# KatanaMajesty/Nebulae

Hardware: AMD Instinct MI355X
Metric: denoised frames/s (1920x1080: GI 1 spp + SVGF temporal + a-trous) (higher is better)
Workload: dtype f32

## Files before the change

### nebulae_amd/csrc/gi.hip

```cpp
#include "gi_device.h"

namespace neb {

#ifndef NEB_SORT_BITS
#define NEB_SORT_BITS 16
#endif
constexpr int kSortBits = NEB_SORT_BITS;
static_assert(kSortBits >= 1 && kSortBits <= 16, "raysort.hip sorts at most two 8-bit digits");

__device__ __forceinline__ uint32_t bounce_sort_key(float3 o, float3 d, const float* smin, const float* sinv)
{
    const uint32_t oct = (d.x < 0.f ? 1u : 0u) | (d.y < 0.f ? 2u : 0u) | (d.z < 0.f ? 4u : 0u);
    const uint32_t key = (oct << (kSortBits - 3)) | (morton30(o, smin, sinv) >> (30 - (kSortBits - 3)));
    return min(key, (1u << kSortBits) - 2u);
}

struct GiRecords {
    float4* ray_o;
    float4* ray_d;
    float4* hit;
    float4* path;
    float4* state;
    float4* srec;
};
constexpr int kSrO = 0, kSrD = 1, kSrContrib = 2, kSrSum = 3;

struct GiArgs {
    SceneView S;
    neb_gi_constants c;
    GiRecords R;
    const uint32_t* albedo;
    const uint32_t* rough_metal;
    const uint2* world_pos;
    const uint2* normal;
    float4* radiance;
    neb_gi_hit* hits;
    unsigned long long* ray_counter;
    uint32_t* bounce_counts;
    uint32_t* shadow_counts;
    uint32_t* table_counts;
    uint32_t sun_table;
    uint32_t hint_pairs;
    uint32_t W, row_begin, row0, row1, tiles_x;
    uint32_t sample;
    uint32_t bounce;
    uint32_t stats;
    uint32_t defer_resolve;
    const uint32_t* tile_order;
    uint32_t* sort_keys;
    uint32_t* sort_vals;
    const uint32_t* sort_order;
    uint32_t* bsort_keys;
    uint32_t* bsort_vals;
    uint32_t raygen_only;
    float4* list;
    uint32_t* list_counts;
    uint32_t list_cap, list_set;
    float smin[3], sinv[3];
    uint32_t first_px, n_px;
};
template <uint32_t RUNS>
__device__ __forceinline__ uint32_t gi_block()
{
    if constexpr (RUNS == 0u)
        return blockIdx.x;
    const uint32_t seg_len = ((gridDim.x + RUNS - 1u) / RUNS + 7u) & ~7u;
    const uint32_t seg = blockIdx.x / seg_len, b = blockIdx.x - seg * seg_len;
    const uint32_t n = min(seg_len, gridDim.x - seg * seg_len);
    const uint32_t q = n >> 3, r = n & 7u, xcd = b & 7u, k = b >> 3;
    return seg * seg_len + (xcd < r ? xcd * (q + 1u) + k : r * (q + 1u) + (xcd - r) * q + k);
}
constexpr uint32_t kShadeRuns = 16u, kRaygenRuns = 16u;
constexpr uint32_t kListSegments = 128u;
#ifndef NEB_LIST_QUAD_BELOW
#define NEB_LIST_QUAD_BELOW 1500000u
#endif
#ifndef NEB_LIST_WAVES
#define NEB_LIST_WAVES 6
#endif

template <uint32_t RUNS = 0u>
__device__ __forceinline__ bool gi_pixel(const GiArgs& a, uint32_t& x, uint32_t& y, size_t& i)
{
    const uint32_t lane = threadIdx.x;
    const uint32_t blk = gi_block<RUNS>();
    const uint32_t tile_x = blk % a.tiles_x, tile_y = blk / a.tiles_x;
    x = tile_x * 8 + (lane & 7);
    y = a.row0 + tile_y * 8 + (lane >> 3);
    i = (size_t)(y - a.row_begin) * a.W + x;
    return x < a.W && y < a.row1;
}

__device__ __forceinline__ void count_rays(uint32_t* block_counts, uint32_t mine, uint32_t slot)
{
    uint32_t total = mine;
#pragma unroll
    for (int off = 32; off > 0; off >>= 1)
        total += __shfl_down(total, off);
    if ((threadIdx.x & 63u) == 0 && total)
        block_counts[slot] += total;
}
__device__ __forceinline__ void count_rays(uint32_t* block_counts, uint32_t mine) { count_rays(block_counts, mine, blockIdx.x); }

#ifndef NEB_RG_STACK
#define NEB_RG_STACK 12
#endif
constexpr int kRgStack = NEB_RG_STACK;
static_assert(32 * (kRgStack * 256 + 1024) <= 160 * 1024 || NEB_TRACE_WAVES < 8, "LDS budget of the closest-hit pass: 32 waves per CU of stacks and child slots in 160 KB");
__global__ __launch_bounds__(64, NEB_TRACE_WAVES) void gi_raygen_trace_kernel(GiArgs a)
{
    __shared__ int stack_mem[kRgStack * 64];
    __shared__ __attribute__((aligned(16))) int child_slot_mem[256];
// ... 74 lines not shown
    count_rays(a.bounce_counts, rays);
    if (a.stats) {
#pragma unroll
        for (int k = 0; k < 5; ++k) {
            uint32_t v = wave_stamp[k];
#pragma unroll
            for (int off = 32; off > 0; off >>= 1)
                v = max(v, (uint32_t)__shfl_xor((int)v, off));
            if (lane == 0)
                atomicAdd(a.ray_counter + 6 + k, (unsigned long long)v);
        }
        if (lane == 0)
            atomicAdd(a.ray_counter + 5, 1ull);
    }
}

__global__ __launch_bounds__(64, NEB_TRACE_WAVES) void gi_bounce_trace_kernel(GiArgs a)
{
    __shared__ int stack_mem[kLdsStack * 64];
    uint32_t x, y;
    size_t i = 0;
    bool active;
    if (a.sort_order) {
        const uint32_t j = blockIdx.x * 64u + threadIdx.x;
        active = j < a.n_px;
        if (active)
            i = a.sort_order[j];
    } else {
        active = gi_pixel(a, x, y, i);
    }
    uint32_t rays = 0;
    if (active) {
        const float4 rd = a.R.ray_d[i];
        if (rd.w != 0.0f) {
            const float4 ro = a.R.ray_o[i];
            Hit hit;
            rays = 1;
            float4 h = make_float4(-1.0f, 0.f, 0.f, 0.f);
            if (traverse(a.S, f3(ro.x, ro.y, ro.z), f3(rd.x, rd.y, rd.z), ro.w, kTraceMax, false, stack_mem + threadIdx.x, hit))
                h = make_float4(hit.t, hit.u, hit.v, __uint_as_float(hit.tri));
            a.R.hit[i] = h;
        }
    }
    if (a.bounce > 1)
        count_rays(a.bounce_counts, rays);
}

struct ShadeOut {
    float4 rec_o = {0.f, 0.f, 0.f, 0.f}, shadow_d = {0.f, 0.f, 0.f, 0.f} , rec_c = {0.f, 0.f, 0.f, 0.f}, sum = {0.f, 0.f, 0.f, 0.f};
    uint32_t rays = 0;
    uint32_t table = 0;
};

template <bool FAST, bool STAGED>
__device__ __forceinline__ void shade_pixel(const GiArgs& a, size_t i, const float4 h, ShadeOut& o, const float4* staged, uint32_t staged_swz)
{
    const float4 pth = a.R.path[i];
    const float4 rd = a.R.ray_d[i];
    const uint32_t trav_iters = a.stats ? __float_as_uint(a.R.srec[4 * i + kSrContrib].w) : 0u;
    float3 throughput = f3(pth.x, pth.y, pth.z);
    if (!(a.sample == 0 && a.bounce == 1))
        o.sum = a.R.srec[4 * i + kSrSum];
    float4 next_d = make_float4(0.f, 0.f, 0.f, 0.f);
    neb_gi_hit dbg = {-1.0f, ~0u, ~0u, 0u};
    const bool alive = rd.w != 0.0f;
    if (alive && h.x == -1.0f) {
        o.sum.x += a.c.skyColor[0] * throughput.x;
        o.sum.y += a.c.skyColor[1] * throughput.y;
        o.sum.z += a.c.skyColor[2] * throughput.z;
    } else if (alive && h.x >= 0.0f) {
        const uint32_t tri = __float_as_uint(h.w);
        Surface surf;
        uint32_t geom;
        TriShade ts;
        if constexpr (STAGED)
            ts = load_tri_shade_at(staged, staged_swz);
        else
            ts = load_tri_shade(a.S, tri);
        const bool shaded = reconstruct_surface<FAST>(a.S, ts, h.y, h.z, surf, geom);
        dbg.t = h.x;
        dbg.geometry = geom;
        if (a.hits)
            dbg.primitive = __float_as_uint(a.S.shade[8 * (size_t)tri + 7].x);
        if (shaded) {
            const float4 ro = a.R.ray_o[i];
            const float3 org = f3(ro.x, ro.y, ro.z), dir = f3(rd.x, rd.y, rd.z);
            const float3 hitP = org + dir * h.x;
            const float3 V = normalize3<FAST>(-dir);
            uint32_t rng = __float_as_uint(pth.w);
            const float a0 = rand01(rng), a1 = rand01(rng);
            const float angle = a0 * 2.0f * 3.1415926535f, dist = fsqrt<false>(a1);
            const float3 sun_dir = f3(a.c.sunLightDirection[0], a.c.sunLightDirection[1], a.c.sunLightDirection[2]);
            const float3 sun_rad = f3(a.c.sunLightRadiance[0], a.c.sunLightRadiance[1], a.c.sunLightRadiance[2]);
            const float3 L = normalize3<false>(-sun_dir);
            const float3 Bv = normalize3<false>(perpendicular(L));
            const float3 T = cross3(Bv, L);
            float sn_a, cs_a;
            det_sincosf(angle, sn_a, cs_a);
            const float3 inc = normalize3<false>(L + (Bv * sn_a + T * cs_a) * a.c.sunTanHalfAngle * dist);
            const bool transition = dot3(surf.GN, inc) <= 0.0f;
            const float3 so = hitP + (transition ? -surf.GN : surf.GN) * 1e-2f;
            const float3 O = evaluate_direct_brdf<FAST>(surf, V, L) * sun_rad * throughput;
            o.rays = 1;
            const uint32_t side = transition ? 1u : 0u;
            bool hinted_hit = false;
            if (a.sun_table && !((ts.lit >> side) & 1u) && ts.hint_side == side && ts.hint[0] != kNoHint) {
                float tt, uu, vv;
#pragma unroll
                for (int pair = 0; pair < kHints && !hinted_hit; pair += 2) {
                    const uint32_t h0 = ts.hint[pair];
                    if (h0 == kNoHint || (uint32_t)pair >= 2u * a.hint_pairs)
                        break;
                    const uint32_t h1 = ts.hint[pair + 1] != kNoHint ? ts.hint[pair + 1] : h0;
                    const float4 a0 = a.S.tris[3 * h0], b0 = a.S.tris[3 * h0 + 1], c0 = a.S.tris[3 * h0 + 2];
                    const float4 a1 = a.S.tris[3 * h1], b1 = a.S.tris[3 * h1 + 1], c1 = a.S.tris[3 * h1 + 2];
                    hinted_hit = intersect_tri_regs(a0, b0, c0, so, inc, 0.001f, kTraceMax, tt, uu, vv) ||
                                 intersect_tri_regs(a1, b1, c1, so, inc, 0.001f, kTraceMax, tt, uu, vv);
                }
            }
            if (hinted_hit) {
                o.table = 1;
            } else if (a.sun_table && ((ts.lit >> side) & 1u)) {
                o.sum.x += O.x;
                o.sum.y += O.y;
                o.sum.z += O.z;
                o.table = 1;
                dbg.flags |= 1u;
            } else {
                o.rec_o = make_float4(so.x, so.y, so.z, 0.001f);
                o.shadow_d = make_float4(inc.x, inc.y, inc.z, 1.0f);
                o.rec_c = make_float4(O.x, O.y, O.z, 0.f);
            }
            if (a.bounce + 1 < a.c.maxPathVertices) {
                uint32_t rng_copy = rng;
                const float3 SNn = normalize3<FAST>(surf.SN);
                const float e0 = rand01(rng_copy), e1 = rand01(rng_copy);
                const float3 Ld = cosine_hemisphere_aligned<FAST>(e0, e1, SNn);
                const float pdiff = 1.0f - specular_probability<FAST>(saturate1(dot3(V, SNn)), specular_f0(surf.albedo, surf.metalness), surf.albedo);
                const float3 no = hitP + surf.GN * 1e-2f;
                throughput = throughput * (surf.albedo * (1.0f - surf.metalness));
                if (rand01(rng) < pdiff)
                    throughput = f3(fdiv<FAST>(throughput.x, pdiff), fdiv<FAST>(throughput.y, pdiff), fdiv<FAST>(throughput.z, pdiff));
                a.R.ray_o[i] = make_float4(no.x, no.y, no.z, 0.001f);
                next_d = make_float4(Ld.x, Ld.y, Ld.z, 1.0f);
                a.R.path[i] = make_float4(throughput.x, throughput.y, throughput.z, __uint_as_float(rng));
            }
            if (a.sample + 1 < a.c.samplesPerPixel)
                a.R.state[i] = make_float4(V.x, V.y, V.z, __uint_as_float(rng));
        }
    }
    if (a.bounce + 1 < a.c.maxPathVertices)
        a.R.ray_d[i] = next_d;
    if (a.sort_keys) {
        uint32_t key = (1u << kSortBits) - 1u;
        if (o.shadow_d.w != 0.0f) {
            key = min(morton30(f3(o.rec_o.x, o.rec_o.y, o.rec_o.z), a.smin, a.sinv) >> (30 - kSortBits), (1u << kSortBits) - 2u);
        }
        a.sort_keys[i] = key;
        a.sort_vals[i] = (uint32_t)i;
    }
    if (a.bsort_keys) {
        uint32_t key = (1u << kSortBits) - 1u;
        if (next_d.w != 0.0f) {
            const float4 no4 = a.R.ray_o[i];
            key = bounce_sort_key(f3(no4.x, no4.y, no4.z), f3(next_d.x, next_d.y, next_d.z), a.smin, a.sinv);
        }
        a.bsort_keys[i] = key;
        a.bsort_vals[i] = (uint32_t)i;
    }
    if (a.hits && a.bounce == 1) {
        if (a.stats)
            dbg.flags |= min(trav_iters, 4095u) << 8;
        a.hits[i] = dbg;
    }
}

template <bool FAST>
__global__ __launch_bounds__(64, NEB_SHADE_WAVES) void gi_shade_kernel(GiArgs a)
{
    uint32_t x, y;
    size_t i;
    const bool active = gi_pixel<kShadeRuns>(a, x, y, i);
    ShadeOut o;
    float4 h = make_float4(-2.0f, 0.f, 0.f, 0.f);
    if (active)
        h = a.R.hit[i];
    __shared__ float4 smem[64 * 8];
    const uint32_t lane = threadIdx.x;
    const bool has_hit = active && h.x >= 0.0f;
    const uint32_t my_tri = has_hit ? __float_as_uint(h.w) : ~0u;
#pragma unroll
    for (uint32_t it = 0; it < 8; ++it) {
        const uint32_t src = it * 8u + (lane >> 3);
        const uint32_t t = (uint32_t)__shfl((int)my_tri, (int)src);
        if (t != ~0u) {
            const float4* g = a.S.shade + 8 * (size_t)t + ((lane & 7u) ^ (src & 7u));
            __builtin_amdgcn_global_load_lds((const __attribute__((address_space(1))) void*)g, (__attribute__((address_space(3))) void*)(smem + it * 64u), 16, 0, 0);
        }
    }
    __syncthreads();
    if (active)
        shade_pixel<FAST, true>(a, i, h, o, smem + lane * 8u, lane & 7u);
    if (a.list) {
        const bool trace = active && o.shadow_d.w != 0.0f;
        const bool final_vertex = a.sample + 1 == a.c.samplesPerPixel && a.bounce + 1 >= a.c.maxPathVertices && !a.defer_resolve;
        if (active && !trace) {
            if (final_vertex) {
                if (o.sum.x != 0.0f || o.sum.y != 0.0f || o.sum.z != 0.0f) {
                    const float inv_spp = 1.0f / (float)a.c.samplesPerPixel;
                    float4 r = a.radiance[i];
                    r.x += o.sum.x * inv_spp;
                    r.y += o.sum.y * inv_spp;
                    r.z += o.sum.z * inv_spp;
                    a.radiance[i] = r;
                }
            } else {
                a.R.srec[4 * i + kSrSum] = o.sum;
            }
        }
        const unsigned long long m = __ballot(trace);
        if (m) {
            const uint32_t seg = blockIdx.x % kListSegments;
            uint32_t base = 0;
            if (lane == 0)
                base = atomicAdd(a.list_counts + a.list_set * kListSegments + seg, (uint32_t)__popcll(m));
            base = (uint32_t)__shfl((int)base, 0);
            if (trace) {
                const uint32_t slot = base + (uint32_t)__popcll(m & ((1ull << lane) - 1ull));
                float4* rec = a.list + 4 * ((size_t)seg * a.list_cap + slot);
                rec[kSrO] = make_float4(o.rec_o.x, o.rec_o.y, o.rec_o.z, __uint_as_float((uint32_t)i));
                rec[kSrD] = o.shadow_d;
                rec[kSrContrib] = o.rec_c;
                rec[kSrSum] = o.sum;
            }
        }
        count_rays(a.shadow_counts, o.rays);
        count_rays(a.table_counts, o.table);
        return;
    }
    __syncthreads();
    float4* xpose = smem;
    xpose[lane * 4 + kSrO] = o.rec_o;
    xpose[lane * 4 + kSrD] = o.shadow_d;
    xpose[lane * 4 + kSrContrib] = o.rec_c;
    xpose[lane * 4 + kSrSum] = o.sum;
    __syncthreads();
    const uint32_t blk = gi_block<kShadeRuns>();
    const uint32_t tile_x = blk % a.tiles_x, tile_y = blk / a.tiles_x;
#pragma unroll
    for (uint32_t k = 0; k < 4; ++k) {
        const uint32_t row = 2 * k + (lane >> 5), col = (lane & 31u) >> 2, comp = lane & 3u;
        const uint32_t px = tile_x * 8 + col, py = a.row0 + tile_y * 8 + row;
        if (px < a.W && py < a.row1)
            a.R.srec[4 * ((size_t)(py - a.row_begin) * a.W + px) + comp] = xpose[(row * 8 + col) * 4 + comp];
    }
    count_rays(a.shadow_counts, o.rays);
    count_rays(a.table_counts, o.table);
}

__device__ __forceinline__ void shadow_wave(const GiArgs& a, size_t i, bool valid, int* stack_mem)
{
    float4* stage = reinterpret_cast<float4*>(stack_mem);
    const uint32_t lane = threadIdx.x;
// ... 356 lines not shown
    GiState::DispatchSet& ds = g->sets[phase == 1 ? (g->begun & 1u) : phase == 2 ? (g->finished & 1u) : g->defer_resolve == 2 ? (g->traces & 1u) : 0u];
    if (g->debug_hits && !g->d_hits) {
        void* p = nullptr;
        GI_HIP(ctx, hipMalloc(&p, npx * sizeof(neb_gi_hit)));
        GI_HIP(ctx, hipMemset(p, 0, npx * sizeof(neb_gi_hit)));
        g->allocs.push_back(p);
        g->d_hits = (neb_gi_hit*)p;
    }
    if (!ds.d_records) {
        void* p = nullptr;
        GI_HIP(ctx, hipMalloc(&p, npx * sizeof(float4) * 9));
        g->allocs.push_back(p);
        ds.d_records = (float4*)p;
    }
    GiArgs a;
    a.S = g->view;
    a.c = *c;
    a.R.ray_o = ds.d_records;
    a.R.ray_d = ds.d_records + npx;
    a.R.hit = ds.d_records + 2 * npx;
    a.R.path = ds.d_records + 3 * npx;
    a.R.state = ds.d_records + 4 * npx;
    a.R.srec = ds.d_records + 5 * npx;
    a.albedo = (const uint32_t*)ctx->planes[NEB_PLANE_ALBEDO][0];
    a.rough_metal = (const uint32_t*)ctx->planes[NEB_PLANE_ROUGH_METAL][0];
    a.world_pos = (const uint2*)ctx->planes[NEB_PLANE_WORLDPOS][0];
    a.normal = (const uint2*)ctx->planes[NEB_PLANE_NORMAL][ctx->cur];
    a.radiance = (float4*)ctx->planes[NEB_PLANE_RADIANCE][ctx->cur];
    a.hits = g->debug_hits ? g->d_hits : nullptr;
    a.ray_counter = g->d_ray_counter;
    a.W = ctx->W;
    a.row_begin = ctx->row_begin;
    a.row0 = row0;
    a.row1 = row1;
    a.tiles_x = (ctx->W + 7) / 8;
    a.stats = g->debug_hits ? 1u : 0u;
    a.sort_keys = a.sort_vals = nullptr;
    a.sort_order = nullptr;
    a.tile_order = (g->d_tile_order && g->tile_order_n == a.tiles_x * ((row1 - row0 + 7) / 8)) ? g->d_tile_order : nullptr;
    a.first_px = (uint32_t)((size_t)(row0 - ctx->row_begin) * ctx->W);
    a.n_px = (uint32_t)((size_t)(row1 - row0) * ctx->W);
    for (int q = 0; q < 3; ++q) {
        a.smin[q] = g->scene_min[q];
        a.sinv[q] = 1.0f / fmaxf(g->scene_max[q] - g->scene_min[q], 1e-20f);
    }
    a.bsort_keys = a.bsort_vals = nullptr;
    a.raygen_only = 0;
    if (phase != 1) {
        GI_HIP(ctx, gi_sun_table_update(g, *c, (hipStream_t)stream));
        GI_HIP(ctx, gi_sun_table_order(g, (hipStream_t)stream));
        g->last_dispatch_stream = (hipStream_t)stream;
        g->last_dispatch_stream_set = true;
    }
    a.sun_table = g->sun_table_state == 1 ? 1u : 0u;
    a.hint_pairs = (uint32_t)g->sun_hints / 2u;
    int tail_slot = -1;
    bool tail_warm = false;
    if (a.sun_table && g->compact_shadow && g->tail_tune && phase != 1) {
        if (g->tail_phase == 3 && hipEventQuery(g->tail_ev[1]) == hipSuccess && hipEventQuery(g->tail_ev[3]) == hipSuccess) {
            float ms_lists = 0.f, ms_sorted = 0.f;
            if (hipEventElapsedTime(&ms_lists, g->tail_ev[0], g->tail_ev[1]) == hipSuccess && hipEventElapsedTime(&ms_sorted, g->tail_ev[2], g->tail_ev[3]) == hipSuccess) {
                g->tail_us[0] = ms_lists * 1e3f, g->tail_us[1] = ms_sorted * 1e3f;
                g->tail_sorted = ms_sorted < 0.95f * ms_lists;
            }
            g->tail_phase = 0;
        } else if (g->tail_phase == 1 && !ds.d_list) {
        } else if (g->tail_phase == 2 && !ds.d_sort && (g->sort_shadow_auto ? a.n_px >= 1500000u : g->sort_shadow)) {
            tail_warm = true;
        } else if (g->tail_phase == 1 || g->tail_phase == 2) {
            tail_slot = g->tail_phase == 1 ? 0 : 2;
            for (int k = 0; k < 2; ++k)
                if (!g->tail_ev[tail_slot + k])
                    GI_HIP(ctx, hipEventCreate(&g->tail_ev[tail_slot + k]));
            g->tail_phase++;
        }
        (void)hipGetLastError();
    }
    const bool compact = a.sun_table && g->compact_shadow && !tail_warm && (tail_slot >= 0 ? tail_slot == 0 : !g->tail_sorted);
    const bool sort_shadow = !compact && (g->sort_shadow_auto ? a.n_px >= 1500000u : g->sort_shadow);
    if (sort_shadow || g->sort_bounce) {
        if (!ds.d_sort) {
            void* p = nullptr;
            GI_HIP(ctx, hipMalloc(&p, 8 * npx * sizeof(uint32_t)));
            g->allocs.push_back(p);
            ds.d_sort = (uint32_t*)p;
            const size_t bytes = ray_sort_scratch_bytes(npx);
            GI_HIP(ctx, hipMalloc(&p, bytes));
            g->allocs.push_back(p);
            ds.d_sort_temp = p;
            g->sort_temp_bytes = bytes;
        }
        if (sort_shadow) {
            a.sort_keys = ds.d_sort;
            a.sort_vals = ds.d_sort + npx;
        }
        if (g->sort_bounce) {
            a.bsort_keys = ds.d_sort + 4 * npx;
            a.bsort_vals = ds.d_sort + 5 * npx;
            a.raygen_only = 1;
        }
    }
    a.defer_resolve = g->defer_resolve ? 1u : 0u;
    ds.pending_spp = c->samplesPerPixel;
    ds.pending_row0 = row0;
    ds.pending_row1 = row1;
    if (g->defer_resolve == 2)
// ... 487 lines not shown
```

### nebulae_amd/csrc/gi_build.hip

```cpp
#include <cstring>
#include <rocprim/device/device_radix_sort.hpp>
#include <rocprim/device/device_scan.hpp>

#include <algorithm>
#include <chrono>
#include <cstdlib>

#include "gi_device.h"

namespace neb {

void gi_on_resize(GiState* g)
{
    if (!g)
        return;
    std::vector<void*> stale = {g->d_hits, g->d_direct_counts};
    for (GiState::DispatchSet& ds : g->sets) {
        for (void* p : {(void*)ds.d_records, (void*)ds.d_block_counts, (void*)ds.d_sort, ds.d_sort_temp, (void*)ds.d_list})
            stale.push_back(p);
        ds = GiState::DispatchSet{};
    }
    g->traces = g->resolves = 0;
    g->begun = g->finished = 0;
    for (void* p : stale) {
// ... 1166 lines not shown
        if (standalone[i]) {
            if (table_entries + (size_t)dtexs[i].w * dtexs[i].h > 0xfffffffeull) {
                delete g;
                return gi_fail(ctx, NEB_ERR_OUT_OF_RANGE, "neb_gi_set_scene: more than 2^32 texels in standalone texture tables");
            }
            dtexs[i].offset = (uint32_t)table_entries;
            table_entries += (size_t)dtexs[i].w * dtexs[i].h;
        }
    g->texture_table_bytes = table_entries * 16 + bundle_entries * 32;
    {
        uint32_t* d_raw = nullptr;
        uint4* d_tables = nullptr;
        uint4* d_bundles = nullptr;
        hipError_t te = hipSuccess;
        auto talloc = [&](void** p, size_t bytes, bool keep) {
            if (te != hipSuccess)
                return;
            te = hipMalloc(p, bytes ? bytes : 16);
            if (te == hipSuccess && keep)
                g->allocs.push_back(*p);
        };
        talloc((void**)&d_raw, raw_total * 4, false);
        talloc((void**)&d_tables, table_entries * 16, true);
        talloc((void**)&d_bundles, bundle_entries * 32, true);
        for (uint32_t i = 0; i < n_texs && te == hipSuccess; ++i)
            te = hipMemcpy(d_raw + raw_off[i], texs[i].rgba8, (size_t)texs[i].width * texs[i].height * 4, hipMemcpyHostToDevice);
        for (uint32_t i = 0; i < n_texs && te == hipSuccess; ++i)
            if (standalone[i]) {
                const size_t n_pos = (size_t)dtexs[i].w * dtexs[i].h;
                hipLaunchKernelGGL(texture_footprints_kernel, dim3((unsigned)((n_pos + 255) / 256)), dim3(256), 0, nullptr, d_raw + raw_off[i],
                                   dtexs[i].w, dtexs[i].h, d_tables + dtexs[i].offset, 1u);
                te = hipGetLastError();
            }
        for (uint32_t i = 0; i < n_mats && te == hipSuccess; ++i) {
            const DevMat& d = dmats[i];
            if (!d.bundle_w)
                continue;
            const size_t n_pos = (size_t)d.bundle_w * d.bundle_h;
            hipLaunchKernelGGL(material_bundle_kernel, dim3((unsigned)((n_pos + 255) / 256)), dim3(256), 0, nullptr, d_raw + raw_off[d.tex[0]],
                               d_raw + raw_off[d.tex[1]], d_raw + raw_off[d.tex[2]], d.bundle_w, d.bundle_h, d_bundles + 2 * (size_t)d.bundle);
            te = hipGetLastError();
        }
        if (te == hipSuccess)
            te = hipDeviceSynchronize();
        if (d_raw)
            (void)hipFree(d_raw);
        if (te != hipSuccess) {
            gi_destroy(g);
            return gi_fail(ctx, NEB_ERR_HIP, "neb_gi_set_scene: texture tables", te);
        }
        g->view.texels = reinterpret_cast<const uint32_t*>(d_tables);
        g->view.bundles = d_bundles;
    }
    g->n_tris = (uint32_t)(g->h_tris.size() / 12);
    memcpy(g->scene_min, smin, sizeof(smin));
    memcpy(g->scene_max, smax, sizeof(smax));
    hipError_t e = hipSuccess;
    if ((e = upload(g, dgeoms, &g->view.geoms)) != hipSuccess || (e = upload(g, dmats, &g->view.mats)) != hipSuccess ||
        (e = upload(g, dtexs, &g->view.texs)) != hipSuccess || (e = upload(g, indices, &g->view.indices)) != hipSuccess ||
        (e = upload(g, normals, &g->view.normals)) != hipSuccess || (e = upload(g, uvs, &g->view.uvs)) != hipSuccess ||
        (e = upload(g, tangents, &g->view.tangents)) != hipSuccess) {
        gi_destroy(g);
        return gi_fail(ctx, NEB_ERR_HIP, "neb_gi_set_scene: upload", e);
    }
    void* ctr = nullptr;
    if ((e = hipMalloc(&ctr, 16 * sizeof(unsigned long long))) != hipSuccess || (e = hipMemset(ctr, 0, 16 * sizeof(unsigned long long))) != hipSuccess) {
        gi_destroy(g);
        return gi_fail(ctx, NEB_ERR_HIP, "neb_gi_set_scene: counter", e);
    }
    g->allocs.push_back(ctr);
    g->d_ray_counter = (unsigned long long*)ctr;
    g->view.n_tris = g->n_tris;
    ctx->gi = g;
    return NEB_OK;
}

#ifndef NEB_SPLIT_AREA_FACTOR
#define NEB_SPLIT_AREA_FACTOR 16.0
#endif
constexpr double kSplitAreaFactor = NEB_SPLIT_AREA_FACTOR, kSplitBudget = 0.25;

struct HostRef {
    uint32_t tri;
    float lo[3], hi[3];
    bool clipped;
};

static double half_area(const float lo[3], const float hi[3])
{
    const double dx = (double)hi[0] - lo[0], dy = (double)hi[1] - lo[1], dz = (double)hi[2] - lo[2];
    return dx * dy + dy * dz + dz * dx;
}

static bool clipped_bounds(const float* t, const float lo[3], const float hi[3], float out_lo[3], float out_hi[3])
{
    double poly[16][3], tmp[16][3];
    int n = 3;
    for (int c = 0; c < 3; ++c) {
        poly[0][c] = t[c];
        poly[1][c] = (double)t[c] + t[3 + c];
        poly[2][c] = (double)t[c] + t[6 + c];
    }
    for (int axis = 0; axis < 3 && n > 0; ++axis)
        for (int side = 0; side < 2 && n > 0; ++side) {
            const double plane = side == 0 ? (double)lo[axis] : (double)hi[axis], sgn = side == 0 ? 1.0 : -1.0;
            int m = 0;
            for (int i = 0; i < n; ++i) {
                const int j = (i + 1) % n;
                const double di = sgn * (poly[i][axis] - plane), dj = sgn * (poly[j][axis] - plane);
                if (di >= 0.0) {
                    for (int c = 0; c < 3; ++c)
                        tmp[m][c] = poly[i][c];
                    ++m;
                }
// ... 469 lines not shown
```

### nebulae_amd/csrc/gi_device.h

```cpp
#pragma once
#pragma clang fp contract(off)

#include "gi_internal.h"

namespace neb {

__device__ __forceinline__ float3 f3(float x, float y, float z) { return make_float3(x, y, z); }
__device__ __forceinline__ float3 operator+(float3 a, float3 b) { return f3(a.x + b.x, a.y + b.y, a.z + b.z); }
__device__ __forceinline__ float3 operator-(float3 a, float3 b) { return f3(a.x - b.x, a.y - b.y, a.z - b.z); }
__device__ __forceinline__ float3 operator*(float3 a, float s) { return f3(a.x * s, a.y * s, a.z * s); }
__device__ __forceinline__ float3 operator*(float3 a, float3 b) { return f3(a.x * b.x, a.y * b.y, a.z * b.z); }
__device__ __forceinline__ float3 operator-(float3 a) { return f3(-a.x, -a.y, -a.z); }
__device__ __forceinline__ float dot3(float3 a, float3 b) { return a.x * b.x + a.y * b.y + a.z * b.z; }
__device__ __forceinline__ float3 cross3(float3 a, float3 b)
{
    return f3(a.y * b.z - a.z * b.y, a.z * b.x - a.x * b.z, a.x * b.y - a.y * b.x);
}
template <bool FAST> __device__ __forceinline__ float fdiv(float a, float b) { return FAST ? a * __builtin_amdgcn_rcpf(b) : a / b; }
template <bool FAST> __device__ __forceinline__ float fsqrt(float x) { return FAST ? __builtin_amdgcn_sqrtf(x) : sqrtf(x); }
__device__ __forceinline__ void det_sincosf(float x, float& s, float& c)
{
    const float k = rintf(x * 0.636619772367581343f);
    float r = fmaf(-k, 1.57079637050628662109375f, x);
    r = fmaf(-k, -4.37113900018624283e-8f, r);
// ... 83 lines not shown
    int e;
    const float m = frexpf(f, &e);
    e -= 1;
    if (e > 15)
        return max_bits;
    if (e < -14)
        return (uint32_t)rintf(ldexpf(f, 14 + mbits));
    const float q = rintf(ldexpf(2.0f * m - 1.0f, mbits));
    const uint32_t bits = ((uint32_t)(e + 15) << mbits) + (uint32_t)q;
    return bits > max_bits ? max_bits : bits;
}
__device__ __forceinline__ float3 unpack_r11g11b10(uint32_t v)
{
    return f3(small_float_decode(v & 0x7ffu, 6), small_float_decode((v >> 11) & 0x7ffu, 6),
              small_float_decode((v >> 22) & 0x3ffu, 5));
}

__device__ __forceinline__ float luminance3(float3 c) { return c.x * 0.2126f + c.y * 0.7152f + c.z * 0.0722f; }
__device__ __forceinline__ float3 specular_f0(float3 albedo, float metal)
{
    return f3(lerp1(0.04f, albedo.x, metal), lerp1(0.04f, albedo.y, metal), lerp1(0.04f, albedo.z, metal));
}
template <bool FAST = false> __device__ __forceinline__ float3 fresnel_schlick(float3 f0, float vdoth)
{
    const float k = 1.0f - fpow5<FAST>(vdoth);
    return f3(f0.x + (1.0f - f0.x) * k, f0.y + (1.0f - f0.y) * k, f0.z + (1.0f - f0.z) * k);
}
template <bool FAST = false> __device__ __forceinline__ float specular_probability(float vdotn, float3 f0, float3 albedo)
{
    const float dr = luminance3(albedo);
    const float fres = saturate1(luminance3(fresnel_schlick<FAST>(f0, saturate1(vdotn))));
    const float diff = dr * (1.0f - fres);
    const float p = fdiv<FAST>(diff, fmaxf(0.0001f, fres + diff));
    return fminf(fmaxf(p, 0.1f), 0.9f);
}
template <bool FAST = false> __device__ __forceinline__ float3 cosine_hemisphere_aligned(float u0, float u1, float3 sn)
{
    const float a = fsqrt<FAST>(u0), b = kPiTwo * u1;
    float sb, cb;
    det_sincosf(b, sb, cb);
    const float3 z = f3(a * cb, a * sb, fsqrt<FAST>(1.0f - u0));
    const float3 up = fabsf(sn.z) < 0.999f ? f3(0, 0, 1) : f3(1, 0, 0);
    const float3 tx = normalize3<FAST>(cross3(up, sn));
    const float3 ty = cross3(sn, tx);
    return normalize3<FAST>(tx * z.x + ty * z.y + sn * z.z);
}
__device__ __forceinline__ float3 perpendicular(float3 u)
{
    const float3 a = f3(fabsf(u.x), fabsf(u.y), fabsf(u.z));
    const uint32_t xm = ((a.x - a.y) < 0 && (a.x - a.z) < 0) ? 1 : 0;
    const uint32_t ym = (a.y - a.z) < 0 ? (1 ^ xm) : 0;
    const uint32_t zm = 1 ^ (xm | ym);
    return cross3(u, f3((float)xm, (float)ym, (float)zm));
}

struct Surface {
    float3 GN, SN, albedo;
    float roughness, metalness;
};

template <bool FAST = false> __device__ float3 evaluate_direct_brdf(const Surface& s, float3 V, float3 L)
{
    const float3 N = s.SN;
    const float3 Hv = normalize3<FAST>(V + L);
    const float LdotN = dot3(L, N), VdotH = saturate1(dot3(V, Hv)), VdotN = dot3(V, N), NdotH = dot3(N, Hv);
    const float3 F0 = specular_f0(s.albedo, s.metalness);
    const float3 F = fresnel_schlick<FAST>(F0, saturate1(VdotH));
    const float3 Kd = f3(1.0f - F.x, 1.0f - F.y, 1.0f - F.z);
    const float3 diff = Kd * (s.albedo * kPiInv);
    const float vn = saturate1(VdotN), ln = saturate1(LdotN), nh = saturate1(NdotH);
    float3 spec = f3(0, 0, 0);
    const float den = 4.0f * vn * ln;
    if (den > 0.0f) {
        const float alpha = s.roughness * s.roughness;
        const float a2 = alpha * alpha;
        const float dd = (nh * nh) * (a2 - 1.0f) + 1.0f;
        const float ndf = fdiv<FAST>(a2, kPi * dd * dd);
        const float k = alpha * 0.5f;
        const float gv = vn * fdiv<FAST>(1.0f, vn * (1.0f - k) + k);
        const float gl = ln * fdiv<FAST>(1.0f, ln * (1.0f - k) + k);
        const float c = ndf * (gv * gl);
        const float inv = fdiv<FAST>(1.0f, den);
        spec = f3(c * F.x * inv, c * F.y * inv, c * F.z * inv);
    }
    return diff + spec;
}

#ifndef NEB_LDS_STACK
#define NEB_LDS_STACK 16
#endif
constexpr int kLdsStack = NEB_LDS_STACK;
constexpr int kSpillStack = 64 - kLdsStack;
static_assert((kLdsStack + kSpillStack) / 3 == 21, "GiState::max_bvh_depth assumes a 64-entry traversal stack");

struct Hit {
    float t, u, v;
    uint32_t tri;
    uint32_t node_visits, tri_tests;
    uint32_t w_iters, w_node_iters, w_node_lanes, w_leaf_iters, w_leaf_lanes;
    uint32_t top_visits[4], deep_sp;
};

__device__ __forceinline__ bool intersect_tri_regs(float4 a, float4 b, float4 c, float3 o, float3 d, float tmin, float tmax, float& t,
                                                   float& u, float& v)
{
    const float3 v0 = f3(a.x, a.y, a.z), e1 = f3(a.w, b.x, b.y), e2 = f3(b.z, b.w, c.x);
// ... 425 lines not shown
            };
            const float a = un(top.x, top.y), b = un(top.z, top.w), cc = un(bot.x, bot.y), dd = un(bot.z, bot.w);
            const float tp = a + fx * (b - a), bt = cc + fx * (dd - cc);
            ch[c] = tp + fy * (bt - tp);
        }
        out.albedo = make_float4(ch[0], ch[1], ch[2], 0.0f);
        out.normal = make_float4(ch[3], ch[4], ch[5], 0.0f);
        out.rm = make_float4(0.0f, ch[6], ch[7], 0.0f);
        return;
    }
    if (m.tex[0] >= 0)
        out.albedo = sample_texture<FAST>(S, m.tex[0], u, v);
    if (m.tex[1] >= 0)
        out.normal = sample_texture<FAST>(S, m.tex[1], u, v);
    if (m.tex[2] >= 0)
        out.rm = sample_texture<FAST>(S, m.tex[2], u, v);
}

__device__ __forceinline__ float3 load3(const float* p, uint32_t i) { return f3(p[3 * i], p[3 * i + 1], p[3 * i + 2]); }
__device__ __forceinline__ float3 xform_dir(const float* m, float3 p)
{
    return f3(p.x * m[0] + p.y * m[3] + p.z * m[6], p.x * m[1] + p.y * m[4] + p.z * m[7], p.x * m[2] + p.y * m[5] + p.z * m[8]);
}

struct TriShade {
    float3 n0, n1, n2;
    float2 uv0, uv1, uv2;
    float4 t0, t1, t2;
    uint32_t geom;
    uint32_t lit;
    uint32_t hint[kHints], hint_side;
};
template <typename Ptr> __device__ __forceinline__ TriShade load_tri_shade_at(Ptr r, uint32_t swz)
{
    const float4 r0 = r[0 ^ swz], r1 = r[1 ^ swz], r2 = r[2 ^ swz], r6 = r[6 ^ swz];
    TriShade t;
    t.n0 = f3(r0.x, r0.y, r0.z);
    t.n1 = f3(r1.x, r1.y, r1.z);
    t.n2 = f3(r2.x, r2.y, r2.z);
    t.uv0 = make_float2(r0.w, r1.w);
    t.uv1 = make_float2(r2.w, r6.x);
    t.uv2 = make_float2(r6.y, r6.z);
    t.geom = __float_as_uint(r6.w) & kGeomMask;
    t.lit = __float_as_uint(r6.w) >> kLitShift;
    t.t0 = r[3 ^ swz];
    t.t1 = r[4 ^ swz];
    t.t2 = r[5 ^ swz];
    const float4 r7 = r[7 ^ swz];
    unpack_hints(r7, t.hint, t.hint_side);
    return t;
}
__device__ __forceinline__ TriShade load_tri_shade(const SceneView& S, uint32_t tri) { return load_tri_shade_at(S.shade + 8 * (size_t)tri, 0u); }

template <bool FAST = false> __device__ __forceinline__ bool reconstruct_surface(const SceneView& S, const TriShade& ts, float bu, float bv, Surface& out, uint32_t& geom)
{
    geom = ts.geom;
    const DevGeom g = S.geoms[geom];
    const float b0 = 1.0f - (bu + bv), b1 = bu, b2 = bv;
    if (!g.valid)
        return false;
    const float3 n0 = ts.n0, n1 = ts.n1, n2 = ts.n2;
    const float3 gn = normalize3<FAST>(f3(n0.x * b0 + n1.x * b1 + n2.x * b2, n0.y * b0 + n1.y * b1 + n2.y * b2, n0.z * b0 + n1.z * b1 + n2.z * b2));
    out.GN = normalize3<FAST>(xform_dir(g.m, gn));
    const float u = ts.uv0.x * b0 + ts.uv1.x * b1 + ts.uv2.x * b2;
    const float v = ts.uv0.y * b0 + ts.uv1.y * b1 + ts.uv2.y * b2;
    if (g.material < 0)
        return false;
    const DevMat m = S.mats[g.material];
    MapSamples maps;
    sample_material_maps<FAST>(S, m, u, v, maps);
    if (m.tex[0] < 0) {
        out.albedo = f3(m.albedo[0], m.albedo[1], m.albedo[2]);
    } else {
        const float4 t = maps.albedo;
        out.albedo = f3(t.x, t.y, t.z);
    }
    if (m.tex[1] < 0) {
        out.SN = out.GN;
    } else {
        float tg[4];
        tg[0] = ts.t0.x * b0 + ts.t1.x * b1 + ts.t2.x * b2;
        tg[1] = ts.t0.y * b0 + ts.t1.y * b1 + ts.t2.y * b2;
        tg[2] = ts.t0.z * b0 + ts.t1.z * b1 + ts.t2.z * b2;
        tg[3] = ts.t0.w * b0 + ts.t1.w * b1 + ts.t2.w * b2;
        const float l4 = fsqrt<FAST>(tg[0] * tg[0] + tg[1] * tg[1] + tg[2] * tg[2] + tg[3] * tg[3]);
#pragma unroll
        for (int k = 0; k < 4; ++k)
            tg[k] = fdiv<FAST>(tg[k], l4);
        const float3 T = f3(tg[0], tg[1], tg[2]);
        const float3 B = normalize3<FAST>(cross3(out.GN, T) * tg[3]);
        const float4 t = maps.normal;
        const float3 N = f3(t.x * 2.0f - 1.0f, t.y * 2.0f - 1.0f, t.z * 2.0f - 1.0f);
        out.SN = normalize3<FAST>(T * N.x + B * N.y + out.GN * N.z);
    }
    if (m.tex[2] < 0) {
        out.roughness = m.rough;
        out.metalness = m.metal;
    } else {
        const float4 t = maps.rm;
        out.roughness = t.y;
        out.metalness = t.z;
    }
    return true;
}

__device__ __forceinline__ uint32_t expand_bits10(uint32_t v)
{
    v = (v * 0x00010001u) & 0xFF0000FFu;
    v = (v * 0x00000101u) & 0x0F00F00Fu;
    v = (v * 0x00000011u) & 0xC30C30C3u;
    v = (v * 0x00000005u) & 0x49249249u;
    return v;
}

__device__ __forceinline__ uint32_t morton30(float3 p, const float* smin, const float* sinv)
{
    const uint32_t qx = (uint32_t)fminf(fmaxf((p.x - smin[0]) * sinv[0] * 1024.0f, 0.0f), 1023.0f);
    const uint32_t qy = (uint32_t)fminf(fmaxf((p.y - smin[1]) * sinv[1] * 1024.0f, 0.0f), 1023.0f);
    const uint32_t qz = (uint32_t)fminf(fmaxf((p.z - smin[2]) * sinv[2] * 1024.0f, 0.0f), 1023.0f);
    return (expand_bits10(qx) << 2) | (expand_bits10(qy) << 1) | expand_bits10(qz);
}
// ... 3 lines not shown
```

### nebulae_amd/csrc/gi_internal.h

```cpp
#pragma once
#include <cmath>
#include <cstdio>
#include <cstring>
#include <vector>

#include "neb_device.h"
#include "neb_internal.h"

namespace neb {


struct DevGeom {
    float m[9];
    int32_t material;
    uint32_t firstIndex;
    uint32_t vertexBase;
    uint32_t valid;
    uint32_t pad[3];
};
struct DevMat {
    int32_t tex[3];
    float albedo[3];
    float rough, metal;
    uint32_t bundle;
    uint32_t bundle_w, bundle_h;
    uint32_t pad;
};
struct DevTex {
    uint32_t offset;
    uint32_t w, h, pad;
};
struct BvhNode {
    float c0min[3];
    int32_t c0;
    float c0max[3];
    int32_t c1;
    float c1min[3];
    uint32_t pad0;
    float c1max[3];
    uint32_t pad1;
};

struct Bvh4Node {
    float4 lox, loy, loz;
    int4 child;
    float4 hix, hiy, hiz;
    int4 pad;
};
static_assert(sizeof(Bvh4Node) == 128 && offsetof(Bvh4Node, hix) == offsetof(Bvh4Node, lox) + 64, "node layout");
struct Bvh4NodeQ {
    float ox, oy, oz, sx;
    float sy, sz;
    uint32_t qlox, qloy;
    uint32_t qloz, qhix, qhiy, qhiz;
    int4 child;
};
static_assert(sizeof(Bvh4NodeQ) == 64, "quantised node layout");
#ifndef NEB_TRACE_WAVES
#define NEB_TRACE_WAVES 8
#endif
#ifndef NEB_SHADE_WAVES
#define NEB_SHADE_WAVES 4
#endif
#ifndef NEB_LEAF_BATCH
#define NEB_LEAF_BATCH 12
#endif
constexpr int kLeafBatch = NEB_LEAF_BATCH;
#ifndef NEB_MAX_LEAF_TRIS
#define NEB_MAX_LEAF_TRIS 2
#endif
constexpr int kMaxLeafTris = NEB_MAX_LEAF_TRIS;
constexpr uint32_t kLitShift = 30u, kGeomMask = (1u << kLitShift) - 1u;
constexpr int kHints = 4;
constexpr uint32_t kNoHint = 0x7fffffu;
__host__ __device__ inline void pack_hints(const uint32_t hint[kHints], uint32_t side, float4& r7)
{
    uint32_t h[kHints];
    for (int k = 0; k < kHints; ++k)
        h[k] = hint[k] < kNoHint ? hint[k] : kNoHint;
    const unsigned long long lo = (unsigned long long)h[0] | ((unsigned long long)h[1] << 23) | ((unsigned long long)(h[2] & 0x3ffffu) << 46);
    union { uint32_t u; float f; } y, z, w;
    y.u = (uint32_t)lo;
    z.u = (uint32_t)(lo >> 32);
    w.u = (h[2] >> 18) | (h[3] << 5) | (side << 31);
    r7.y = y.f, r7.z = z.f, r7.w = w.f;
}
__host__ __device__ inline void unpack_hints(const float4& r7, uint32_t hint[kHints], uint32_t& side)
{
    union { float f; uint32_t u; } y, z, w;
    y.f = r7.y, z.f = r7.z, w.f = r7.w;
    const unsigned long long lo = (unsigned long long)y.u | ((unsigned long long)z.u << 32);
    hint[0] = (uint32_t)lo & kNoHint;
    hint[1] = (uint32_t)(lo >> 23) & kNoHint;
    hint[2] = ((uint32_t)(lo >> 46) | (w.u << 18)) & kNoHint;
    hint[3] = (w.u >> 5) & kNoHint;
    side = w.u >> 31;
}

struct SceneView {
    const float4* tris;
    const Bvh4Node* nodes;
    const Bvh4NodeQ* qnodes;
    const DevGeom* geoms;
    const DevMat* mats;
    const DevTex* texs;
    const uint32_t* indices;
    const float* normals;
    const float* uvs;
    const float* tangents;
    const uint32_t* texels;
    const uint4* bundles;
    const float4* shade;
    uint32_t n_tris;
    int32_t root;
    uint32_t n_qnodes;
};

struct GiState {
    SceneView view{};
    std::vector<void*> allocs;
    std::vector<float> h_tris;
    float scene_min[3] = {0, 0, 0}, scene_max[3] = {0, 0, 0};
    uint32_t n_tris = 0, n_nodes = 0, bvh_depth = 0, build_passes = 0;
    float build_ms = 0.f;
    size_t texture_table_bytes = 0;
    uint32_t max_bvh_depth = 21;
    bool built = false;
    unsigned long long* d_ray_counter = nullptr;
    neb_gi_hit* d_hits = nullptr;
    bool debug_hits = false;
    struct DispatchSet {
        float4* d_records = nullptr;
        uint32_t* d_sort = nullptr;
        void* d_sort_temp = nullptr;
        uint32_t* d_block_counts = nullptr;
        uint32_t* d_list = nullptr;
        uint32_t list_epoch = 0;
        uint32_t pending_spp = 1, pending_row0 = 0, pending_row1 = 0;
        bool awaiting_resolve = false;
        uint32_t resolve_seq = 0;
        neb_gi_constants split_c{};
        uint32_t split_row0 = 0, split_row1 = 0;
    } sets[2];
    uint32_t resolve_seq = 0;
    uint32_t* d_tile_order = nullptr;
    uint32_t tile_order_n = 0, tile_order_cap = 0;
    uint32_t traces = 0, resolves = 0;
    uint32_t begun = 0, finished = 0;
    uint32_t* d_direct_counts = nullptr;
    unsigned long long last_stats[16] = {};
    int defer_resolve = 0;
    bool exact_shade = false;
    bool sort_shadow = true;
    bool sort_shadow_auto = true;
    bool sort_bounce = false;
    size_t sort_temp_bytes = 0;
    size_t n_block_counts = 0;
    bool sun_table = true;
    int sun_table_state = 0;
    float sun_table_pending[4] = {0, 0, 0, 0};
    uint32_t sun_hold = 2, sun_seen = 0, sun_table_age = 0;
    int sun_hold_option = 0;
    float sun_table_key[4] = {0, 0, 0, 0};
    unsigned long long* d_sun_counts = nullptr;
    uint32_t* d_sun_hint_list = nullptr;
    uint32_t sun_hint_list_cap = 0;
    uint32_t sun_table_builds = 0;
    hipEvent_t sun_table_event = nullptr;
    hipEvent_t sun_build_ev[2] = {nullptr, nullptr};
    hipStream_t sun_table_stream = nullptr;
    bool sun_table_event_pending = false;
    hipStream_t last_dispatch_stream = nullptr;
// ... 56 lines not shown
```

Measured before the change: 1640.

## Flatten geometry+material into one header and hoist shade-kernel loads

Builds a per-geometry 128-byte ShadeHeader that merges the geometry transform and its material, so shading reads it with six vector loads instead of two dependent loads (geom, then material). Path, ray direction, origin, radiance and the first hint-triangle pair are loaded earlier in the shade kernel so their latency overlaps with other work. The sun basis (L, B, T) is now computed once on the host and passed in the kernel arguments instead of per pixel. The cost is extra register pressure from the hoisted loads and a larger argument struct.

New measurement: 1702, median of 6. 1.04x the previous value.

```diff
diff --git a/nebulae_amd/csrc/gi.hip b/nebulae_amd/csrc/gi.hip
--- a/nebulae_amd/csrc/gi.hip
+++ b/nebulae_amd/csrc/gi.hip
@@ -58,6 +58,8 @@
     uint32_t list_cap, list_set;
     float smin[3], sinv[3];
     uint32_t first_px, n_px;
+    const ShadeHeader* heads;
+    float sun_L[3], sun_B[3], sun_T[3];
 };
 template <uint32_t RUNS>
 __device__ __forceinline__ uint32_t gi_block()
@@ -238,11 +240,10 @@
     uint32_t table = 0;
 };
 
-template <bool FAST, bool STAGED>
-__device__ __forceinline__ void shade_pixel(const GiArgs& a, size_t i, const float4 h, ShadeOut& o, const float4* staged, uint32_t staged_swz)
-{
-    const float4 pth = a.R.path[i];
-    const float4 rd = a.R.ray_d[i];
+template <bool FAST>
+__device__ __forceinline__ void shade_pixel(const GiArgs& a, size_t i, const float4 h, const float4 pth, const float4 rd, const float4 ro, ShadeOut& o,
+                                            const float4* staged, uint32_t staged_swz)
+{
     const uint32_t trav_iters = a.stats ? __float_as_uint(a.R.srec[4 * i + kSrContrib].w) : 0u;
     float3 throughput = f3(pth.x, pth.y, pth.z);
     if (!(a.sample == 0 && a.bounce == 1))
@@ -257,30 +258,29 @@
     } else if (alive && h.x >= 0.0f) {
         const uint32_t tri = __float_as_uint(h.w);
         Surface surf;
-        uint32_t geom;
-        TriShade ts;
-        if constexpr (STAGED)
-            ts = load_tri_shade_at(staged, staged_swz);
-        else
-            ts = load_tri_shade(a.S, tri);
-        const bool shaded = reconstruct_surface<FAST>(a.S, ts, h.y, h.z, surf, geom);
+        const TriShade ts = load_tri_shade_at(staged, staged_swz);
+        const ShadeHead head = load_shade_header(a.heads, ts.geom);
+        const bool hint_fetch = a.sun_table && a.hint_pairs && !((ts.lit >> ts.hint_side) & 1u) && ts.hint[0] != kNoHint;
+        float4 ha0 = make_float4(0.f, 0.f, 0.f, 0.f), hb0 = ha0, hc0 = ha0, ha1 = ha0, hb1 = ha0, hc1 = ha0;
+        if (hint_fetch) {
+            const uint32_t h0 = ts.hint[0], h1 = ts.hint[1] != kNoHint ? ts.hint[1] : h0;
+            ha0 = a.S.tris[3 * h0], hb0 = a.S.tris[3 * h0 + 1], hc0 = a.S.tris[3 * h0 + 2];
+            ha1 = a.S.tris[3 * h1], hb1 = a.S.tris[3 * h1 + 1], hc1 = a.S.tris[3 * h1 + 2];
+        }
+        const bool shaded = reconstruct_surface<FAST>(a.S, head, ts, h.y, h.z, surf);
         dbg.t = h.x;
-        dbg.geometry = geom;
+        dbg.geometry = ts.geom;
         if (a.hits)
             dbg.primitive = __float_as_uint(a.S.shade[8 * (size_t)tri + 7].x);
         if (shaded) {
-            const float4 ro = a.R.ray_o[i];
             const float3 org = f3(ro.x, ro.y, ro.z), dir = f3(rd.x, rd.y, rd.z);
             const float3 hitP = org + dir * h.x;
             const float3 V = normalize3<FAST>(-dir);
             uint32_t rng = __float_as_uint(pth.w);
             const float a0 = rand01(rng), a1 = rand01(rng);
             const float angle = a0 * 2.0f * 3.1415926535f, dist = fsqrt<false>(a1);
-            const float3 sun_dir = f3(a.c.sunLightDirection[0], a.c.sunLightDirection[1], a.c.sunLightDirection[2]);
             const float3 sun_rad = f3(a.c.sunLightRadiance[0], a.c.sunLightRadiance[1], a.c.sunLightRadiance[2]);
-            const float3 L = normalize3<false>(-sun_dir);
-            const float3 Bv = normalize3<false>(perpendicular(L));
-            const float3 T = cross3(Bv, L);
+            const float3 L = f3(a.sun_L[0], a.sun_L[1], a.sun_L[2]), Bv = f3(a.sun_B[0], a.sun_B[1], a.sun_B[2]), T = f3(a.sun_T[0], a.sun_T[1], a.sun_T[2]);
             float sn_a, cs_a;
             det_sincosf(angle, sn_a, cs_a);
             const float3 inc = normalize3<false>(L + (Bv * sn_a + T * cs_a) * a.c.sunTanHalfAngle * dist);
@@ -297,6 +297,11 @@
                     const uint32_t h0 = ts.hint[pair];
                     if (h0 == kNoHint || (uint32_t)pair >= 2u * a.hint_pairs)
                         break;
+                    if (pair == 0) {
+                        hinted_hit = intersect_tri_regs(ha0, hb0, hc0, so, inc, 0.001f, kTraceMax, tt, uu, vv) ||
+                                     intersect_tri_regs(ha1, hb1, hc1, so, inc, 0.001f, kTraceMax, tt, uu, vv);
+                        continue;
+                    }
                     const uint32_t h1 = ts.hint[pair + 1] != kNoHint ? ts.hint[pair + 1] : h0;
                     const float4 a0 = a.S.tris[3 * h0], b0 = a.S.tris[3 * h0 + 1], c0 = a.S.tris[3 * h0 + 2];
                     const float4 a1 = a.S.tris[3 * h1], b1 = a.S.tris[3 * h1 + 1], c1 = a.S.tris[3 * h1 + 2];
@@ -369,8 +374,16 @@
     const bool active = gi_pixel<kShadeRuns>(a, x, y, i);
     ShadeOut o;
     float4 h = make_float4(-2.0f, 0.f, 0.f, 0.f);
-    if (active)
+    const bool final_vertex = a.sample + 1 == a.c.samplesPerPixel && a.bounce + 1 >= a.c.maxPathVertices && !a.defer_resolve;
+    float4 pth = make_float4(0.f, 0.f, 0.f, 0.f), rd = pth, ro = pth, rad = pth;
+    if (active) {
         h = a.R.hit[i];
+        pth = a.R.path[i];
+        rd = a.R.ray_d[i];
+        ro = a.R.ray_o[i];
+        if (a.list && final_vertex)
+            rad = a.radiance[i];
+    }
     __shared__ float4 smem[64 * 8];
     const uint32_t lane = threadIdx.x;
     const bool has_hit = active && h.x >= 0.0f;
@@ -386,15 +399,14 @@
     }
     __syncthreads();
     if (active)
-        shade_pixel<FAST, true>(a, i, h, o, smem + lane * 8u, lane & 7u);
+        shade_pixel<FAST>(a, i, h, pth, rd, ro, o, smem + lane * 8u, lane & 7u);
     if (a.list) {
         const bool trace = active && o.shadow_d.w != 0.0f;
-        const bool final_vertex = a.sample + 1 == a.c.samplesPerPixel && a.bounce + 1 >= a.c.maxPathVertices && !a.defer_resolve;
         if (active && !trace) {
             if (final_vertex) {
                 if (o.sum.x != 0.0f || o.sum.y != 0.0f || o.sum.z != 0.0f) {
                     const float inv_spp = 1.0f / (float)a.c.samplesPerPixel;
-                    float4 r = a.radiance[i];
+                    float4 r = rad;
                     r.x += o.sum.x * inv_spp;
                     r.y += o.sum.y * inv_spp;
                     r.z += o.sum.z * inv_spp;
@@ -857,6 +869,8 @@
         g->last_dispatch_stream = (hipStream_t)stream;
         g->last_dispatch_stream_set = true;
     }
+    a.heads = g->shade_heads;
+    sun_frame(c->sunLightDirection, a.sun_L, a.sun_B, a.sun_T);
     a.sun_table = g->sun_table_state == 1 ? 1u : 0u;
     a.hint_pairs = (uint32_t)g->sun_hints / 2u;
     int tail_slot = -1;
diff --git a/nebulae_amd/csrc/gi_build.hip b/nebulae_amd/csrc/gi_build.hip
--- a/nebulae_amd/csrc/gi_build.hip
+++ b/nebulae_amd/csrc/gi_build.hip
@@ -1242,6 +1242,23 @@
         g->view.texels = reinterpret_cast<const uint32_t*>(d_tables);
         g->view.bundles = d_bundles;
     }
+    std::vector<ShadeHeader> heads(n_geoms);
+    for (uint32_t gi = 0; gi < n_geoms; ++gi) {
+        ShadeHeader& hd = heads[gi];
+        const DevGeom& d = dgeoms[gi];
+        memset(&hd, 0, sizeof(hd));
+        memcpy(hd.m, d.m, sizeof(hd.m));
+        hd.valid = d.valid;
+        hd.material = d.material;
+        hd.tex[0] = hd.tex[1] = hd.tex[2] = -1;
+        if (d.material >= 0) {
+            const DevMat& mt = dmats[d.material];
+            hd.bundle = mt.bundle, hd.bundle_w = mt.bundle_w, hd.bundle_h = mt.bundle_h;
+            memcpy(hd.tex, mt.tex, sizeof(hd.tex));
+            memcpy(hd.albedo, mt.albedo, sizeof(hd.albedo));
+            hd.rough = mt.rough, hd.metal = mt.metal;
+        }
+    }
     g->n_tris = (uint32_t)(g->h_tris.size() / 12);
     memcpy(g->scene_min, smin, sizeof(smin));
     memcpy(g->scene_max, smax, sizeof(smax));
@@ -1249,7 +1266,7 @@
     if ((e = upload(g, dgeoms, &g->view.geoms)) != hipSuccess || (e = upload(g, dmats, &g->view.mats)) != hipSuccess ||
         (e = upload(g, dtexs, &g->view.texs)) != hipSuccess || (e = upload(g, indices, &g->view.indices)) != hipSuccess ||
         (e = upload(g, normals, &g->view.normals)) != hipSuccess || (e = upload(g, uvs, &g->view.uvs)) != hipSuccess ||
-        (e = upload(g, tangents, &g->view.tangents)) != hipSuccess) {
+        (e = upload(g, tangents, &g->view.tangents)) != hipSuccess || (e = upload(g, heads, &g->shade_heads)) != hipSuccess) {
         gi_destroy(g);
         return gi_fail(ctx, NEB_ERR_HIP, "neb_gi_set_scene: upload", e);
     }
diff --git a/nebulae_amd/csrc/gi_device.h b/nebulae_amd/csrc/gi_device.h
--- a/nebulae_amd/csrc/gi_device.h
+++ b/nebulae_amd/csrc/gi_device.h
@@ -159,6 +159,23 @@
     const uint32_t ym = (a.y - a.z) < 0 ? (1 ^ xm) : 0;
     const uint32_t zm = 1 ^ (xm | ym);
     return cross3(u, f3((float)xm, (float)ym, (float)zm));
+}
+__host__ __device__ inline void sun_frame(const float sun_dir[3], float L[3], float B[3], float T[3])
+{
+    const float nx = -sun_dir[0], ny = -sun_dir[1], nz = -sun_dir[2];
+    const float l = sqrtf(nx * nx + ny * ny + nz * nz);
+    L[0] = nx / l, L[1] = ny / l, L[2] = nz / l;
+    const float ax = fabsf(L[0]), ay = fabsf(L[1]), az = fabsf(L[2]);
+    const uint32_t xm = ((ax - ay) < 0 && (ax - az) < 0) ? 1 : 0;
+    const uint32_t ym = (ay - az) < 0 ? (1 ^ xm) : 0;
+    const uint32_t zm = 1 ^ (xm | ym);
+    const float ex = (float)xm, ey = (float)ym, ez = (float)zm;
+    const float px = L[1] * ez - L[2] * ey, py = L[2] * ex - L[0] * ez, pz = L[0] * ey - L[1] * ex;
+    const float pl = sqrtf(px * px + py * py + pz * pz);
+    B[0] = px / pl, B[1] = py / pl, B[2] = pz / pl;
+    T[0] = B[1] * L[2] - B[2] * L[1];
+    T[1] = B[2] * L[0] - B[0] * L[2];
+    T[2] = B[0] * L[1] - B[1] * L[0];
 }
 
 struct Surface {
@@ -690,10 +707,36 @@
 }
 __device__ __forceinline__ TriShade load_tri_shade(const SceneView& S, uint32_t tri) { return load_tri_shade_at(S.shade + 8 * (size_t)tri, 0u); }
 
-template <bool FAST = false> __device__ __forceinline__ bool reconstruct_surface(const SceneView& S, const TriShade& ts, float bu, float bv, Surface& out, uint32_t& geom)
-{
-    geom = ts.geom;
-    const DevGeom g = S.geoms[geom];
+struct ShadeHead {
+    float m[9];
+    uint32_t valid;
+    int32_t material;
+    DevMat mat;
+};
+__device__ __forceinline__ ShadeHead load_shade_header(const ShadeHeader* heads, uint32_t geom)
+{
+    const float4* q = reinterpret_cast<const float4*>(heads + geom);
+    const float4 q0 = q[0], q1 = q[1], q2 = q[2], q3 = q[3], q4 = q[4], q5 = q[5];
+    ShadeHead h;
+    h.m[0] = q0.x, h.m[1] = q0.y, h.m[2] = q0.z, h.m[3] = q0.w;
+    h.m[4] = q1.x, h.m[5] = q1.y, h.m[6] = q1.z, h.m[7] = q1.w;
+    h.m[8] = q2.x;
+    h.valid = __float_as_uint(q2.y);
+    h.material = (int32_t)__float_as_uint(q2.z);
+    h.mat.bundle = __float_as_uint(q2.w);
+    h.mat.bundle_w = __float_as_uint(q3.x);
+    h.mat.bundle_h = __float_as_uint(q3.y);
+    h.mat.tex[0] = (int32_t)__float_as_uint(q3.z);
+    h.mat.tex[1] = (int32_t)__float_as_uint(q3.w);
+    h.mat.tex[2] = (int32_t)__float_as_uint(q4.x);
+    h.mat.albedo[0] = q4.y, h.mat.albedo[1] = q4.z, h.mat.albedo[2] = q4.w;
+    h.mat.rough = q5.x, h.mat.metal = q5.y;
+    h.mat.pad = 0;
+    return h;
+}
+
+template <bool FAST = false> __device__ __forceinline__ bool reconstruct_surface(const SceneView& S, const ShadeHead& g, const TriShade& ts, float bu, float bv, Surface& out)
+{
     const float b0 = 1.0f - (bu + bv), b1 = bu, b2 = bv;
     if (!g.valid)
         return false;
@@ -704,7 +747,7 @@
     const float v = ts.uv0.y * b0 + ts.uv1.y * b1 + ts.uv2.y * b2;
     if (g.material < 0)
         return false;
-    const DevMat m = S.mats[g.material];
+    const DevMat& m = g.mat;
     MapSamples maps;
     sample_material_maps<FAST>(S, m, u, v, maps);
     if (m.tex[0] < 0) {
diff --git a/nebulae_amd/csrc/gi_internal.h b/nebulae_amd/csrc/gi_internal.h
--- a/nebulae_amd/csrc/gi_internal.h
+++ b/nebulae_amd/csrc/gi_internal.h
@@ -26,6 +26,18 @@
     uint32_t bundle_w, bundle_h;
     uint32_t pad;
 };
+struct alignas(128) ShadeHeader {
+    float m[9];
+    uint32_t valid;
+    int32_t material;
+    uint32_t bundle;
+    uint32_t bundle_w, bundle_h;
+    int32_t tex[3];
+    float albedo[3];
+    float rough, metal;
+    uint32_t pad[10];
+};
+static_assert(sizeof(ShadeHeader) == 128 && offsetof(ShadeHeader, rough) == 80, "shade header layout (load_shade_header, gi_device.h)");
 struct DevTex {
     uint32_t offset;
     uint32_t w, h, pad;
@@ -118,6 +130,7 @@
 
 struct GiState {
     SceneView view{};
+    const ShadeHeader* shade_heads = nullptr;
     std::vector<void*> allocs;
     std::vector<float> h_tris;
     float scene_min[3] = {0, 0, 0}, scene_max[3] = {0, 0, 0};
```
